# libraz/mygram-db

Hardware: AMD Instinct MI355X
Metric: queries/sec + p50 latency, 10M-doc bigram index, batch=1024 3-term AND (higher is better)
Workload: dtype u32 set algebra + f64 BM25

## Files before the change

### mygram-db_amd/csrc/mgx_api.cpp

```cpp
#include <hip/hip_runtime.h>

#include <dlfcn.h>
#include <pthread.h>

#include <algorithm>
#include <atomic>
#include <chrono>
#include <cmath>
#include <condition_variable>
#include <map>
#include <cstdio>
#include <cstdlib>
#include <cstring>
#include <functional>
#include <memory>
#include <mutex>
#include <string>
#include <thread>
#include <tuple>
#include <unordered_map>
#include <vector>

#include "../../include/mygram_gpu.h"
#include "mgx_highlight.hpp"
// ... 272 lines not shown
    bool operator==(const TableKey& o) const { return row == o.row && idf == o.idf && k1 == o.k1 && b == o.b && avg == o.avg; }
  };
  struct TableKeyHash {
    size_t operator()(const TableKey& k) const {
      uint64_t h = k.row * 0x9E3779B97F4A7C15ull;
      for (uint64_t v : {k.idf, k.k1, k.b, k.avg}) h = (h ^ v) * 0xFF51AFD7ED558CCDull + (h >> 29);
      return static_cast<size_t>(h);
    }
  };
  std::mutex table_mu;
  std::unordered_map<TableKey, uint32_t, TableKeyHash> table_slot;
  DevBuf d_table_pool;
  uint32_t table_cap = 0, table_used = 0, table_dl = 0;
  hipStream_t table_stream = nullptr;
  hipEvent_t table_ev = nullptr;
  mgx::TableJob* job_ring = nullptr;
  DevBuf d_job_ring;
  uint32_t job_ring_at = 0;
  std::vector<mgx::TableJob> pending_jobs;
  hipEvent_t chain_ev = nullptr;
  std::atomic<int> fifo{1};
  bool table_ev_recorded = false;
  static constexpr uint32_t kJobRing = 4096;
  size_t table_doubles() const { return static_cast<size_t>(mgx::kFastPoolTf + 1) * table_dl; }
  struct NormTable {
    uint64_t k1, b, avg;
    DevBuf d;
  };
  std::vector<std::unique_ptr<NormTable>> norm_tables;
  struct BlockMax {
    uint64_t k1, b, avg;
    double step;
    DevBuf d, d_fine;
  };
  std::vector<std::unique_ptr<BlockMax>> block_max;
  std::unordered_map<std::string, uint64_t> df_cache;
  uint32_t n_bitmap_rows = 0, n_fine_rows = 0;
  std::atomic<uint32_t> live_row{mgx::kNoRow};
  std::atomic<bool> bitmaps_clean{false};
  DevBuf d_doc_map;
  DevBuf d_fine_rows;
  std::vector<uint32_t> h_fine_map;
};

namespace mgx {
struct RcclId {
  char internal[128];
};
constexpr int kRcclUint8 = 1, kRcclUint64 = 5, kRcclSum = 0;
static inline uint64_t Bits(double d) {
  uint64_t u;
  std::memcpy(&u, &d, 8);
  return u;
}

static hipError_t SyncDevIndex(mgx_index* idx) {
  if (!idx->d_dev_index.p) {
    ResourceScope none(nullptr);
    hipError_t e = idx->d_dev_index.Alloc(sizeof(DevIndex));
    if (e != hipSuccess) return e;
  }
  return hipMemcpy(idx->d_dev_index.p, &idx->dev, sizeof(DevIndex), hipMemcpyHostToDevice);
}

static uint64_t GetContributionTable(mgx_index* idx, uint32_t bm_row, double idf, double k1, double b, double avgdl) {
  if (idx->table_cap == 0) return 0;
// ... 41 lines not shown
    done += n;
  }
  idx->pending_jobs.clear();
  if ((e = hipEventRecord(idx->table_ev, idx->table_stream)) != hipSuccess) return e;
  idx->table_ev_recorded = true;
  return hipSuccess;
}

static const double* GetLengthNormTable(mgx_index* idx, double k1, double b, double avgdl) {
  std::lock_guard<std::mutex> lock(idx->table_mu);
  for (const auto& t : idx->norm_tables)
    if (t->k1 == Bits(k1) && t->b == Bits(b) && t->avg == Bits(avgdl)) return t->d.as<double>();
  if (idx->norm_tables.size() >= 64) return nullptr;
  double h[256];
  const double one_minus_b = 1.0 - b, avg = std::max(avgdl, 1.0);
  for (uint32_t dli = 0; dli < 256; ++dli) {
    const double length_norm = one_minus_b + b * static_cast<double>(dli) / avg;
    h[dli] = k1 * length_norm;
  }
  auto t = std::make_unique<mgx_index::NormTable>();
  t->k1 = Bits(k1);
  t->b = Bits(b);
  t->avg = Bits(avgdl);
  ResourceScope none(nullptr);
  if (hipSetDevice(idx->device) != hipSuccess || t->d.Alloc(sizeof(h)) != hipSuccess ||
      hipMemcpy(t->d.p, h, sizeof(h), hipMemcpyHostToDevice) != hipSuccess) {
    (void)hipGetLastError();
    return nullptr;
  }
  idx->norm_tables.push_back(std::move(t));
  return idx->norm_tables.back()->d.as<double>();
}

static const uint8_t* GetBlockMax(mgx_index* idx, double k1, double b, double avgdl, double* step, const uint8_t** fine) {
  *fine = nullptr;
  static const bool off = std::getenv("MGX_NO_PRUNE") != nullptr && atoi(std::getenv("MGX_NO_PRUNE")) != 0;
  if (off || !idx->can_score || idx->n_bitmap_rows == 0 || !(k1 > 0.0) || !(b >= 0.0 && b <= 1.0) || !(avgdl >= 0.0))
    return nullptr;
  {
    std::lock_guard<std::mutex> lock(idx->table_mu);
    for (const auto& t : idx->block_max)
      if (t->k1 == Bits(k1) && t->b == Bits(b) && t->avg == Bits(avgdl)) {
        *step = t->step;
        *fine = t->d_fine.as<uint8_t>();
        return t->d.as<uint8_t>();
      }
    if (idx->block_max.size() >= 4) return nullptr;
  }
  const double* ktab = GetLengthNormTable(idx, k1, b, avgdl);
  if (!ktab) return nullptr;
  std::lock_guard<std::mutex> lock(idx->table_mu);
  for (const auto& t : idx->block_max)
    if (t->k1 == Bits(k1) && t->b == Bits(b) && t->avg == Bits(avgdl)) {
      *step = t->step;
      *fine = t->d_fine.as<uint8_t>();
      return t->d.as<uint8_t>();
    }
  auto t = std::make_unique<mgx_index::BlockMax>();
  t->k1 = Bits(k1);
  t->b = Bits(b);
  t->avg = Bits(avgdl);
  t->step = (k1 + 1.0) / 253.0;
  ResourceScope none(nullptr);
  const size_t bytes = static_cast<size_t>(idx->dev.n_tiles) * idx->n_bitmap_rows * 256u;
  if (hipSetDevice(idx->device) != hipSuccess || t->d.Alloc(bytes) != hipSuccess) {
    (void)hipGetLastError();
    return nullptr;
  }
  const size_t fine_bytes = static_cast<size_t>(idx->dev.n_tiles) * idx->n_fine_rows * 1024u;
  if (fine_bytes && t->d_fine.Alloc(fine_bytes) != hipSuccess) {
    (void)hipGetLastError();
    return nullptr;
  }
  if (LaunchBuildBlockMax(idx->dev.tfnib, idx->dev.nib_row_stride, idx->dev.dl8, ktab, k1 + 1.0, 1.0 / t->step, nullptr,
                          idx->n_bitmap_rows, idx->dev.n_tiles, false, t->d.p, idx->stream) != 0 ||
      LaunchBuildBlockMax(idx->dev.tfnib, idx->dev.nib_row_stride, idx->dev.dl8, ktab, k1 + 1.0, 1.0 / t->step,
                          idx->d_fine_rows.as<uint32_t>(), idx->n_fine_rows, idx->dev.n_tiles, true, t->d_fine.p,
                          idx->stream) != 0 ||
      hipStreamSynchronize(idx->stream) != hipSuccess) {
    (void)hipGetLastError();
    return nullptr;
  }
  *step = t->step;
  *fine = t->d_fine.as<uint8_t>();
  idx->block_max.push_back(std::move(t));
  return idx->block_max.back()->d.as<uint8_t>();
}
}


extern "C" {

int mgx_abi_version(void) { return MGX_ABI_VERSION; }
const char* mgx_last_error(void) { return mgx::g_last_error.c_str(); }
void mgx_free(void* p) { std::free(p); }

int mgx_device_count(void) {
  int n = 0;
  if (hipGetDeviceCount(&n) != hipSuccess) {
    (void)hipGetLastError();
    return 0;
  }
  return n;
}


int mgx_columns_build(const mgx_build_params* params, const uint8_t* text_bytes, const uint64_t* text_off,
                      uint32_t first_doc_id, uint64_t n_docs, mgx_columns** out) {
  if (out) *out = nullptr;
  if (!params || !out || !text_off || (n_docs && !text_bytes && text_off[n_docs] != 0))
    return mgx::Fail(MGX_ERR_INVALID_ARGUMENT, "mgx_columns_build: null argument");
  if (params->struct_size < sizeof(mgx_build_params) || params->version != MGX_ABI_VERSION)
    return mgx::Fail(MGX_ERR_INVALID_ARGUMENT, "mgx_columns_build: bad struct_size/version");
  if (static_cast<uint64_t>(first_doc_id) + n_docs > 0xFFFFFFFFull)
    return mgx::Fail(MGX_ERR_OUT_OF_RANGE, "mgx_columns_build: doc ids exceed uint32");
  try {
    mgx::Columns* c = nullptr;
// ... 285 lines not shown
}

void mgx_index_destroy(mgx_index* idx) {
  if (!idx) return;
  (void)hipSetDevice(idx->device);
  if (idx->stream) (void)hipStreamDestroy(idx->stream);
  if (idx->side_stream) (void)hipStreamDestroy(idx->side_stream);
  if (idx->table_stream) {
    (void)hipStreamSynchronize(idx->table_stream);
    (void)hipStreamDestroy(idx->table_stream);
  }
  if (idx->table_ev) (void)hipEventDestroy(idx->table_ev);
  if (idx->job_ring) (void)hipHostFree(idx->job_ring);
  delete idx;
}

int mgx_posting_size(const mgx_index* idx, uint32_t gram_id, uint64_t* out) {
  if (out) *out = 0;
  if (!idx || !out) return mgx::Fail(MGX_ERR_INVALID_ARGUMENT, "mgx_posting_size: null argument");
  if (gram_id >= idx->n_grams) return mgx::Fail(MGX_ERR_OUT_OF_RANGE, "mgx_posting_size: unknown gram id");
  *out = idx->h_offsets[gram_id + 1] - idx->h_offsets[gram_id];
  return MGX_OK;
}

int mgx_index_memory_bytes(const mgx_index* idx, uint64_t* out) {
  if (out) *out = 0;
  if (!idx || !out) return mgx::Fail(MGX_ERR_INVALID_ARGUMENT, "mgx_index_memory_bytes: null argument");
  *out = idx->d_offsets.bytes + idx->d_docids.bytes + idx->d_tf.bytes + idx->d_doc_len.bytes +
         idx->d_skip_row.bytes + idx->d_tile_off.bytes + idx->d_gram_bitmaps.bytes + idx->d_filter_bitmaps.bytes +
         idx->d_text.bytes + idx->d_text_off.bytes + idx->d_dl8.bytes + idx->d_tfnib.bytes + idx->d_table_pool.bytes +
         idx->d_tf_ovf_pos.bytes + idx->d_tf_ovf_val.bytes;
  {
    std::lock_guard<std::mutex> lock(const_cast<mgx_index*>(idx)->table_mu);
    for (const auto& t : idx->block_max) *out += t->d.bytes + t->d_fine.bytes;
    for (const auto& t : idx->norm_tables) *out += t->d.bytes;
  }
  return MGX_OK;
}

int mgx_index_set_batch_order(mgx_index* idx, uint32_t order) {
  if (!idx || order > MGX_ORDER_CONCURRENT) return mgx::Fail(MGX_ERR_INVALID_ARGUMENT, "mgx_index_set_batch_order: bad argument");
  idx->fifo.store(order == MGX_ORDER_FIFO ? 1 : 0);
  return MGX_OK;
}

int mgx_index_attach_text(mgx_index* idx, const uint8_t* text_bytes, const uint64_t* text_off) {
  if (!idx || !text_off) return mgx::Fail(MGX_ERR_INVALID_ARGUMENT, "mgx_index_attach_text: null argument");
  const uint64_t n = idx->dev.n_docs;
  for (uint64_t i = 0; i < n; ++i)
    if (text_off[i + 1] < text_off[i] || text_off[i + 1] - text_off[i] > 0xFFFFFFFFull)
      return mgx::Fail(MGX_ERR_INVALID_ARGUMENT, "mgx_index_attach_text: offsets must ascend");
  const uint64_t total = text_off[n] - text_off[0];
  if (total && !text_bytes) return mgx::Fail(MGX_ERR_INVALID_ARGUMENT, "mgx_index_attach_text: null text");
  std::lock_guard<std::mutex> lock(idx->mu);
  MGX_HIP(hipSetDevice(idx->device));
  std::vector<uint64_t> rel(n + 1);
  for (uint64_t i = 0; i <= n; ++i) rel[i] = text_off[i] - text_off[0];
  MGX_HIP(mgx::Upload(idx->d_text, text_bytes ? text_bytes + text_off[0] : nullptr, total, 128));
  MGX_HIP(mgx::Upload(idx->d_text_off, rel.data(), rel.size()));
  idx->dev.text = idx->d_text.as<uint8_t>();
  idx->dev.text_off = idx->d_text_off.as<uint64_t>();
  uint64_t longest = 0;
  for (uint64_t i = 0; i < n; ++i) longest = std::max<uint64_t>(longest, text_off[i + 1] - text_off[i]);
  idx->max_text_bytes = static_cast<uint32_t>(longest);
  MGX_HIP(mgx::SyncDevIndex(idx));
  return MGX_OK;
}
// ... 1014 lines not shown
    if (f.n_ops == static_cast<uint32_t>(kFastMaxOps) || (op == kOpLoad) != (f.n_ops == 0)) return false;
    FastOp o{};
    uint64_t stride = 0;
    if (lf.kind == kLeafGramBitmap) {
      o.base = reinterpret_cast<uint64_t>(idx->dev.gram_bitmaps + static_cast<uint64_t>(lf.b) * idx->dev.gb_row_stride);
      stride = idx->dev.gb_tile_stride * 8;
    } else if (lf.kind == kLeafFilterBitmap) {
      o.base = static_cast<uint64_t>(lf.b) * idx->dev.fb_row_stride * 8;
      stride = idx->dev.fb_tile_stride * 8;
      o.code |= 16u;
    } else if (lf.kind == kLeafCondBitmap) {
      o.base = reinterpret_cast<uint64_t>(cond_arena + static_cast<uint64_t>(lf.b) * idx->dev.fb_row_stride);
      stride = idx->dev.fb_tile_stride * 8;
    } else {
      return false;
    }
    if (stride > 0xFFFFFFFFull) return false;
    o.tile_stride = static_cast<uint32_t>(stride);
    o.code |= (op == kOpLoad || op == kOpOr) ? kFastOr : op == kOpAnd ? kFastAnd : kFastAndNot;
    f.ops[f.n_ops++] = o;
  }
  if (f.n_ops == 0) return false;
  for (size_t t = 0; t < s.score.size(); ++t) {
    const DevLeaf& lf = s.leaves[s.score[t].leaf];
    if (lf.kind != kLeafGramBitmap) return false;
    FastScore& fs = f.score[t];
    fs.nib = reinterpret_cast<uint64_t>(idx->dev.tfnib + static_cast<uint64_t>(lf.b) * idx->dev.nib_row_stride);
    fs.idf = s.score[t].idf;
    fs.gram = lf.a;
    fs.skip_row = lf.row;
  }
  if (s.reverse != 0) {
    double step = 0.0;
    f.blockmax = GetBlockMax(idx, s.k1, s.b, s.avgdl, &step, &f.blockmax_fine);
    if (f.blockmax) {
      f.bm_tile_stride = idx->n_bitmap_rows * 256u;
      f.bmf_tile_stride = idx->n_fine_rows * 1024u;
      double idf_max = 0.0;
      for (size_t t = 0; t < s.score.size(); ++t) idf_max = std::max(idf_max, s.score[t].idf);
      const double wunit = idf_max > 0.0 ? idf_max * (1.0 + 0x1p-40) / 255.0 : 1.0;
      f.bm_inv_unit = 1.0 / (wunit * step);
      f.bm_wpack = f.bm_w4 = f.bm_cint = 0;
      for (size_t t = 0; t < s.score.size(); ++t) {
        const uint32_t w = static_cast<uint32_t>(std::min(255.0, std::ceil(s.score[t].idf / wunit)));
        if (t < 4) f.bm_wpack |= w << (8 * t); else f.bm_w4 = w;
      }
      for (size_t t = 0; t < s.score.size(); ++t) {
        const DevLeaf& lf = s.leaves[s.score[t].leaf];
        FastScore& fs = f.score[t];
        const uint32_t frow = f.blockmax_fine ? idx->h_fine_map[lf.b] : kNoRow;
        fs.bm_mode = frow != kNoRow ? 2u : 1u;
        fs.bm_off = frow != kNoRow ? frow * 1024u : lf.b * 256u;
      }
    }
  }
  f.n_score = static_cast<uint32_t>(s.score.size());
  f.needed = q.needed;
  f.cap = q.cap;
  f.descending = q.descending;
  f.k1 = q.k1;
  f.b = q.b;
  f.one_minus_b = q.one_minus_b;
  f.k1_plus_1 = q.k1_plus_1;
  f.avgdl_clamped = q.avgdl_clamped;
  return true;
}

static void RouteCandMerge(mgx_batch* b, Group& g, const std::vector<QuerySpec>& specs, const PathSwitches& sw,
                           GroupPlan& p) {
  static const uint64_t kMaxPerTile = std::getenv("MGX_CAND_MAX_PER_TILE") ? static_cast<uint64_t>(atoll(std::getenv("MGX_CAND_MAX_PER_TILE"))) : 64ull;
  const mgx_index* idx = b->idx;
  for (uint32_t i = 0; sw.cand && i < p.n; ++i) {
    const QuerySpec& s = specs[g.qids[i]];
    if (p.route[i] == Route::kFast || !s.flat || s.prog.empty()) continue;
    if (p.score_mode && (!s.fast_score_ok || s.score.empty())) continue;
    bool ok = true, counted = false;
    uint32_t driver = kNoLeaf;
    uint64_t best = ~0ull, longest_list = 0;
    for (size_t pc = 0; ok && pc < s.prog.size(); ++pc) {
      const uint32_t op = s.prog[pc] >> 24, arg = s.prog[pc] & 0xFFFFFFu;
      if (op == kOpCount) {
        counted = true;
        continue;
      }
      if ((op == kOpLoad) != (pc == 0) || (op != kOpLoad && op != kOpAnd && op != kOpAndNot)) { ok = false; break; }
// ... 2559 lines not shown
```

### mygram-db_amd/csrc/mgx_internal.hpp

```cpp
#pragma once

#include <cstdint>

namespace mgx {

constexpr int kBlock = 256;
constexpr int kTileShift = 14;
constexpr uint32_t kTileDocs = 1u << kTileShift;
constexpr int kWordsPerTile = kTileDocs / 64;
constexpr int kMaxTilesPerItem = 64;
constexpr uint32_t kNoRow = 0xFFFFFFFFu;
constexpr uint32_t kMaxLeaves = 192;
constexpr uint32_t kMaxLdsLeaves = 64;
constexpr uint32_t kMaxScoreTerms = 64;
constexpr uint32_t kMaxNeeded = 1024;
constexpr uint32_t kMergeMaxOps = 6;
constexpr uint32_t kMatchBuf = 2048;

enum LeafKind : uint32_t {
  kLeafList = 0,
  kLeafGramBitmap = 1,
  kLeafFilterBitmap = 2,
  kLeafRange = 3,
  kLeafExplicit = 4,
// ... 98 lines not shown
  const uint32_t* tile_off;
  const uint64_t* gram_bitmaps;
  uint64_t gb_tile_stride, gb_row_stride;
  const uint64_t* filter_bitmaps;
  uint64_t fb_tile_stride, fb_row_stride;
  const uint8_t* text;
  const uint64_t* text_off;
  uint32_t first_doc_id;
  uint32_t n_docs;
  uint32_t n_tiles;
  uint32_t max_doc_len;
};

constexpr int kFastMaxOps = 8;
constexpr int kFastMaxScore = 5;
constexpr uint32_t kFastPoolTf = 14;
#ifndef MGX_FWAVES
#define MGX_FWAVES 8
#endif
constexpr int kFastBlock = 64 * MGX_FWAVES;
constexpr int kFastWaves = kFastBlock / 64;

enum FastOpKind : uint32_t { kFastOr = 0, kFastAnd = 1, kFastAndNot = 2 };
struct FastOp {
  uint64_t base;
  uint32_t tile_stride;
  uint32_t code;
};
struct FastScore {
  uint64_t nib;
  double idf;
  uint32_t gram, skip_row;
  uint32_t bm_mode, bm_off;
};
struct DevFastQuery {
  uint32_t n_ops, n_score, needed, cap;
  uint32_t descending, pad0;
  uint32_t pad1, pad1b;
  uint32_t bm_wpack, bm_w4;
  uint32_t bm_cint, pad2;
  double bm_inv_unit;
  double k1, b, one_minus_b, k1_plus_1, avgdl_clamped;
  const uint8_t* blockmax;
  const uint8_t* blockmax_fine;
  uint32_t bm_tile_stride, bmf_tile_stride;
  FastOp ops[kFastMaxOps];
  FastScore score[kFastMaxScore];
};
static_assert(sizeof(DevFastQuery) % 8 == 0, "DevFastQuery is read with scalar loads");

struct FastPlan {
  uint32_t ring;
  uint32_t max_cap;
  uint32_t bytes, pad;
  const double* ktab;
};
struct TableJob {
  double idf, k1, b, avgdl;
  uint32_t slot, pad;
};
FastPlan PlanFast(uint32_t max_cap, const double* ktab);
uint32_t FastTableDl(uint32_t max_doc_len);

struct DevItem {
  uint32_t query, tile_begin, n_tiles, list;
};

struct DevCondition {
  uint64_t literal;
  double eq_epsilon;
  uint32_t op, null_matches, never_matches;
// ... 100 lines not shown
```

### mygram-db_amd/csrc/mgx_kernels.hip

```cpp
#include <hip/hip_runtime.h>

#include <algorithm>
#include <cstdlib>

#include "mgx_fuzzy.hpp"
#include "mgx_internal.hpp"
#include "mgx_launch.hpp"

namespace mgx {

#ifdef MGX_ABLATION
#define MGX_ABLATE(bt, bit) (((bt).debug_skip & (bit)) != 0)
#else
#define MGX_ABLATE(bt, bit) false
#endif


__device__ __forceinline__ int lane_id() { return threadIdx.x & 63; }

__device__ __forceinline__ uint32_t wave_uniform(uint32_t v) { return __builtin_amdgcn_readfirstlane(v); }
__device__ __forceinline__ float wave_uniform(float v) {
  return __uint_as_float(__builtin_amdgcn_readfirstlane(__float_as_uint(v)));
}
__device__ __forceinline__ uint64_t wave_uniform(uint64_t v) {
// ... 116 lines not shown
                                    const uint64_t* __restrict__ row_hi, uint32_t first_doc_id, uint32_t row0,
                                    uint64_t tile_stride, uint64_t row_stride,
                                    unsigned long long* __restrict__ bitmaps) {
  const uint32_t row = blockIdx.y;
  const uint64_t lo = row_lo[row], hi = row_hi[row];
  unsigned long long* bm = bitmaps + static_cast<uint64_t>(row0 + row) * row_stride;
  for (uint64_t p = lo + static_cast<uint64_t>(blockIdx.x) * blockDim.x + threadIdx.x; p < hi;
       p += static_cast<uint64_t>(gridDim.x) * blockDim.x) {
    const uint32_t slot = docids[p] - first_doc_id;
    atomicOr(&bm[static_cast<uint64_t>(slot >> kTileShift) * tile_stride + ((slot >> 6) & (kWordsPerTile - 1))],
             1ull << (slot & 63));
  }
}

__global__ void build_tfnib_kernel(const uint32_t* __restrict__ docids, const uint8_t* __restrict__ tf,
                                   const uint64_t* __restrict__ row_lo, const uint64_t* __restrict__ row_hi,
                                   uint32_t first_doc_id, uint64_t row_stride_bytes, uint8_t* __restrict__ nib) {
  const uint32_t row = blockIdx.y;
  const uint64_t lo = row_lo[row], hi = row_hi[row];
  uint32_t* out = reinterpret_cast<uint32_t*>(nib + static_cast<uint64_t>(row) * row_stride_bytes);
  for (uint64_t p = lo + static_cast<uint64_t>(blockIdx.x) * blockDim.x + threadIdx.x; p < hi;
       p += static_cast<uint64_t>(gridDim.x) * blockDim.x) {
    const uint32_t slot = docids[p] - first_doc_id;
    const uint32_t v = tf[p] < 15 ? tf[p] : 15u;
    atomicOr(&out[slot >> 3], v << ((slot & 7u) * 4u));
  }
}

template <bool kFine>
__global__ __launch_bounds__(256) void build_blockmax_kernel(const uint8_t* __restrict__ nib, uint64_t nib_row_stride,
                                                             const uint8_t* __restrict__ dl8,
                                                             const double* __restrict__ ktab, double k1_plus_1,
                                                             double inv_step, const uint32_t* __restrict__ rows,
                                                             uint32_t n_rows, uint64_t n_out, void* __restrict__ out) {
  const uint64_t idx = static_cast<uint64_t>(blockIdx.x) * blockDim.x + threadIdx.x;
  if (idx >= n_out) return;
  const uint32_t word = static_cast<uint32_t>(idx & 255u);
  const uint64_t tr = idx >> 8;
  const uint32_t r = static_cast<uint32_t>(tr % n_rows);
  const uint32_t row = rows ? rows[r] : r;
  const uint64_t gw = (tr / n_rows) * 256u + word;
  const uint4* np = reinterpret_cast<const uint4*>(nib + static_cast<uint64_t>(row) * nib_row_stride + gw * 32u);
  const uint4* dp = reinterpret_cast<const uint4*>(dl8 + gw * 64u);
  const uint4 n4[2] = {np[0], np[1]};
  const uint4 d4[4] = {dp[0], dp[1], dp[2], dp[3]};
  const uint32_t nw[8] = {n4[0].x, n4[0].y, n4[0].z, n4[0].w, n4[1].x, n4[1].y, n4[1].z, n4[1].w};
  const uint32_t dw[16] = {d4[0].x, d4[0].y, d4[0].z, d4[0].w, d4[1].x, d4[1].y, d4[1].z, d4[1].w,
                           d4[2].x, d4[2].y, d4[2].z, d4[2].w, d4[3].x, d4[3].y, d4[3].z, d4[3].w};
  double best[4] = {0.0, 0.0, 0.0, 0.0};
#pragma unroll
  for (int s = 0; s < 64; ++s) {
    const uint32_t tf = (nw[s >> 3] >> ((s & 7) * 4)) & 15u;
    if (tf == 0u) continue;
    const uint32_t d = (dw[s >> 2] >> ((s & 3) * 8)) & 255u;
    const double tfd = static_cast<double>(tf);
    const double gv = tf == 15u ? k1_plus_1 : tfd * k1_plus_1 / (tfd + ktab[d]);
    best[s >> 4] = gv > best[s >> 4] ? gv : best[s >> 4];
  }
  uint32_t packed = 0, whole = 0;
#pragma unroll
  for (int j = 0; j < 4; ++j) {
    uint32_t qv = 0;
    if (best[j] > 0.0) {
      const double steps = floor(best[j] * inv_step * (1.0 + 0x1p-40));
      qv = steps >= 254.0 ? 255u : static_cast<uint32_t>(steps) + 1u;
    }
    packed |= qv << (8 * j);
    whole = qv > whole ? qv : whole;
  }
  if (kFine) static_cast<uint32_t*>(out)[idx] = packed;
  else static_cast<uint8_t*>(out)[idx] = static_cast<uint8_t>(whole);
}


__device__ __forceinline__ void scatter_segment(const uint32_t* __restrict__ ids, uint64_t lo, uint64_t hi,
                                                uint32_t tile_first_doc, uint32_t* __restrict__ bm32) {
  uint64_t p0 = lo & ~3ull;
  for (uint64_t p = p0 + 4ull * threadIdx.x; p < hi; p += 4ull * kBlock) {
    const uint4 v = *reinterpret_cast<const uint4*>(ids + p);
    const uint32_t e[4] = {v.x, v.y, v.z, v.w};
    uint32_t curw = 0xFFFFFFFFu, curm = 0;
#pragma unroll
    for (int j = 0; j < 4; ++j) {
      uint64_t q = p + j;
      if (q >= lo && q < hi) {
        uint32_t bit = e[j] - tile_first_doc;
        uint32_t w = bit >> 5, m = 1u << (bit & 31);
        if (w == curw) {
          curm |= m;
        } else {
          if (curm) atomicOr(&bm32[curw], curm);
          curw = w;
          curm = m;
        }
      }
    }
    if (curm) atomicOr(&bm32[curw], curm);
  }
}

struct WaveTopK {
  uint64_t* keys;
  uint32_t* docs;
  uint32_t cap, needed;
// ... 1367 lines not shown
__global__ __launch_bounds__(kWaveBlock, 6) void wave_score_lists_kernel(DevIndex ix, DevBatch bt, WavePlan plan) {
  wave_score_body(ix, bt, plan);
}


#ifndef MGX_FPL
#define MGX_FPL 4
#endif
constexpr int kFastPerLane = MGX_FPL;
constexpr uint32_t kFastRound = 64 * kFastPerLane;
constexpr uint32_t kFastPairs = 320;

struct FastOffsets {
  uint32_t ktab, pairs, ring, tk_keys, tk_docs, misc, total;
};
__host__ __device__ inline FastOffsets carve_fast(const FastPlan& p) {
  FastOffsets o;
  uint32_t at = 0;
  o.ktab = at;     at += 256 * 8;
  o.pairs = at;    at += kFastWaves * kFastPairs * 8;
  o.ring = at;     at += kFastWaves * p.ring * 4;
  o.tk_keys = at;  at += kFastWaves * 2 * p.max_cap * 8;
  o.tk_docs = at;  at += kFastWaves * 2 * p.max_cap * 4;
  o.misc = at;     at += 64;
  o.total = at;
  return o;
}
uint32_t FastTableDl(uint32_t max_doc_len) {
  const uint32_t t = max_doc_len + 1 < kTableDlMax ? max_doc_len + 1 : kTableDlMax;
  return (t + 1u) & ~1u;
}
FastPlan PlanFast(uint32_t max_cap, const double* ktab) {
  FastPlan p{};
  p.ring = kFastRound + 128;
  p.max_cap = max_cap;
  p.ktab = ktab;
  p.bytes = carve_fast(p).total;
  return p;
}

typedef uint32_t u32x4 __attribute__((ext_vector_type(4)));
typedef const u32x4 __attribute__((address_space(1)))* gptr_u4;
typedef const uint32_t __attribute__((address_space(1)))* gptr_u1;
typedef const DevFastQuery __attribute__((address_space(4)))* FastQueryPtr;

__device__ __noinline__ uint32_t fast_exact_tf(const DevIndex* ix, uint32_t gram, uint32_t row, uint32_t slot) {
  return exact_tf(*ix, gram, row, slot);
}

template <int T>
__device__ __forceinline__ void fast_load_blockmax(const FastQueryPtr fq, uint32_t tile, uint32_t lane, u32x4 (&raw)[T]) {
  const uint64_t bm = reinterpret_cast<uint64_t>(fq->blockmax), bmf = reinterpret_cast<uint64_t>(fq->blockmax_fine);
  const uint32_t st = fq->bm_tile_stride, stf = fq->bmf_tile_stride;
#pragma unroll
  for (int i = 0; i < T; ++i) {
    const bool fine = fq->score[i].bm_mode == 2u;
    const uint64_t row = (fine ? bmf : bm) + static_cast<uint64_t>(tile) * (fine ? stf : st) + fq->score[i].bm_off;
    const uint32_t off = fine ? lane << 4 : (lane >> 2) << 4;
    raw[i] = *reinterpret_cast<gptr_u4>(row + off);
  }
}

template <int T>
__device__ __forceinline__ uint32_t fast_quarter_mask(const FastQueryPtr fq, uint32_t lane, const u32x4 (&raw)[T],
                                                      uint64_t bound) {
  const uint32_t tint = static_cast<uint32_t>(
      fmin(floor(key_score(bound, true) * fq->bm_inv_unit * (1.0 - 0x1p-30)), 4294967040.0));
  const uint32_t wpack = fq->bm_wpack, w4 = fq->bm_w4, cint = fq->bm_cint;
  uint32_t bmw[T][4];
#pragma unroll
  for (int i = 0; i < T; ++i) {
    bmw[i][0] = raw[i].x;
    bmw[i][1] = raw[i].y;
    bmw[i][2] = raw[i].z;
    bmw[i][3] = raw[i].w;
    const uint32_t mode = fq->score[i].bm_mode;
    if (mode == 1u) {
      const uint32_t l3 = lane & 3u;
      const uint32_t c = l3 == 0u ? raw[i].x : l3 == 1u ? raw[i].y : l3 == 2u ? raw[i].z : raw[i].w;
      bmw[i][0] = __builtin_amdgcn_perm(0u, c, 0x00000000u);
      bmw[i][1] = __builtin_amdgcn_perm(0u, c, 0x01010101u);
      bmw[i][2] = __builtin_amdgcn_perm(0u, c, 0x02020202u);
      bmw[i][3] = __builtin_amdgcn_perm(0u, c, 0x03030303u);
    } else if (mode != 2u) {
      bmw[i][0] = bmw[i][1] = bmw[i][2] = bmw[i][3] = 0;
    }
  }
  uint32_t mk = 0;
#pragma unroll
  for (int k = 0; k < 4; ++k) {
    const uint32_t t0 = bmw[0][k], t1 = T > 1 ? bmw[T > 1 ? 1 : 0][k] : 0u, t2 = T > 2 ? bmw[T > 2 ? 2 : 0][k] : 0u,
                   t3 = T > 3 ? bmw[T > 3 ? 3 : 0][k] : 0u;
    const uint32_t lo01 = __builtin_amdgcn_perm(t1, t0, 0x05010400u), hi01 = __builtin_amdgcn_perm(t1, t0, 0x07030602u);
    const uint32_t lo23 = T > 2 ? __builtin_amdgcn_perm(t3, t2, 0x05010400u) : 0u;
    const uint32_t hi23 = T > 2 ? __builtin_amdgcn_perm(t3, t2, 0x07030602u) : 0u;
    uint32_t qb[4];
    qb[0] = __builtin_amdgcn_perm(lo23, lo01, 0x05040100u);
    qb[1] = __builtin_amdgcn_perm(lo23, lo01, 0x07060302u);
    qb[2] = __builtin_amdgcn_perm(hi23, hi01, 0x05040100u);
    qb[3] = __builtin_amdgcn_perm(hi23, hi01, 0x07060302u);
// ... 33 lines not shown

  WaveTopK tk;
  tk.cap = fq->cap;
  tk.needed = fq->needed;
  tk.lds_sort = true;
  tk.keys = reinterpret_cast<uint64_t*>(smem + fo.tk_keys) + static_cast<size_t>(wave) * 2 * fq->cap;
  tk.docs = reinterpret_cast<uint32_t*>(smem + fo.tk_docs) + static_cast<size_t>(wave) * 2 * fq->cap;
  tk.have = 0;
  tk.pend = 0;
  tk.bound_key = 0;
  tk.bound_doc = 0;
  tk.gbound_ptr = bt.bounds ? bt.bounds + it.query : nullptr;
  tk.gbound = 0;
  for (uint32_t i = lane; i < 2 * tk.cap; i += 64) {
    tk.keys[i] = 0;
    tk.docs[i] = 0;
  }
  __syncthreads();

  __amdgpu_buffer_rsrc_t nib_rsrc[T];
  double idf[T];
#pragma unroll
  for (int i = 0; i < T; ++i) {
    nib_rsrc[i] = __builtin_amdgcn_make_buffer_rsrc(reinterpret_cast<void*>(fq->score[i].nib), 0,
                                                    static_cast<int>((ix.n_docs + 1u) >> 1), 0x00020000);
    idf[i] = fq->score[i].idf;
  }
  const __amdgpu_buffer_rsrc_t dl_rsrc = __builtin_amdgcn_make_buffer_rsrc(
      const_cast<uint8_t*>(ix.dl8), 0, static_cast<int>(ix.n_docs), 0x00020000);
  const double k1_plus_1 = fq->k1_plus_1;
  const bool prune = fq->blockmax != 0;

  uint32_t cnt0 = 0, cnt1 = 0, cnt2 = 0, cnt3 = 0, cnt_res = 0;
  uint32_t pend = 0;
  uint32_t np = 0;

  auto score_round = [&](uint32_t g0, uint32_t n) {
    uint32_t slot[kFastPerLane], dli[kFastPerLane], nb[kFastPerLane][T];
#pragma unroll
    for (int m = 0; m < kFastPerLane; ++m) {
      const uint32_t j = m * 64 + lane;
      slot[m] = j < n ? ring[g0 + j] : 0u;
    }
#pragma unroll
    for (int m = 0; m < kFastPerLane; ++m) {
#pragma unroll
      for (int i = 0; i < T; ++i) nb[m][i] = __builtin_amdgcn_raw_buffer_load_b8(nib_rsrc[i], slot[m] >> 1, 0, 0);
      dli[m] = __builtin_amdgcn_raw_buffer_load_b8(dl_rsrc, slot[m], 0, 0);
    }
#pragma nounroll
    for (int m = 0; m < kFastPerLane; ++m) {
      if (static_cast<uint32_t>(m) * 64u >= n) break;
      uint32_t sl = slot[0], dl = dli[0], nbm[T];
#pragma unroll
      for (int i = 0; i < T; ++i) nbm[i] = nb[0][i];
#pragma unroll
      for (int mm = 1; mm < kFastPerLane; ++mm) {
        if (m == mm) {
          sl = slot[mm];
          dl = dli[mm];
#pragma unroll
          for (int i = 0; i < T; ++i) nbm[i] = nb[mm][i];
        }
      }
      const bool valid = static_cast<uint32_t>(m) * 64u + lane < n;
      double kd = ktab[dl];
      const uint32_t sh = (sl & 1u) << 2;
      uint32_t tf[T], mx = 0;
#pragma unroll
      for (int i = 0; i < T; ++i) {
        tf[i] = (nbm[i] >> sh) & 15u;
        mx = max(mx, tf[i]);
      }
      if (__ballot(valid && (mx == 15u || dl == 255u)) != 0) {
#pragma unroll
        for (int i = 0; i < T; ++i)
          if (valid && tf[i] == 15u) tf[i] = fast_exact_tf(bt.dev_index, fq->score[i].gram, fq->score[i].skip_row, sl);
        if (valid && dl == 255u) {
          const double dld = static_cast<double>(ix.doc_len[sl]);
          kd = fq->k1 * (fq->one_minus_b + fq->b * dld / fq->avgdl_clamped);
        }
      }
      double score = 0.0;
#pragma unroll
      for (int i = 0; i < T; ++i) {
        const double tfd = static_cast<double>(tf[i]);
        const double c = tf[i] != 0u ? idf[i] * (tfd * k1_plus_1) / (tfd + kd) : 0.0;
        score = i == 0 ? c : score + c;
      }
      const uint32_t doc = ix.first_doc_id + sl;
      wave_topk_offer(tk, valid, score_key(score, desc), desc ? doc : ~doc);
    }
  };

  auto load_half = [&](uint32_t o, uint32_t tile, uint32_t h) {
    const uint64_t op_base = fq->ops[o].base;
    const uint32_t op_code = fq->ops[o].code, op_stride = fq->ops[o].tile_stride;
    const uint64_t base = op_base + ((op_code & 16u) ? reinterpret_cast<uint64_t>(ix.filter_bitmaps) : 0ull) +
                          static_cast<uint64_t>(tile) * op_stride;
    const gptr_u4 p = reinterpret_cast<gptr_u4>(base) + lane * 2 + h;
    return p[0];
  };

  for (uint32_t tile = tile_begin + wave;; tile += kFastWaves) {
    const bool flush = tile >= tile_end;
    uint32_t a[8] = {0, 0, 0, 0, 0, 0, 0, 0};
    uint64_t bound = 0;
    if (!flush) {
      wave_topk_refresh_gbound(tk);
      uint32_t qmask = 0xFFFFu;
      if (prune) {
        bound = tk.gbound;
        if (tk.have >= tk.needed && tk.bound_key > bound) bound = tk.bound_key;
      }
      u32x4 raw[T];
#pragma unroll
      for (int i = 0; i < T; ++i) raw[i] = u32x4{0u, 0u, 0u, 0u};
      if (prune) fast_load_blockmax<T>(fq, tile, lane, raw);
      auto combine = [&](int h, uint32_t o, const u32x4 w) {
        const uint32_t code = fq->ops[o].code;
        const uint32_t x[4] = {w.x, w.y, w.z, w.w};
        const uint32_t kind = wave_uniform(code & 15u);
        if (kind == kFastAnd) {
#pragma unroll
          for (int j = 0; j < 4; ++j) a[h * 4 + j] &= x[j];
// ... 79 lines not shown
            }
            np += static_cast<uint32_t>(__popcll(m));
          }
        }
      }
      for (;;) {
        if (np < 64u && !(flush && (np != 0u || pend != 0u))) break;
        const uint32_t take = min(np, 64u);
        wave_lds_sync();
        uint32_t base = 0, bits = 0;
        if (lane < take) {
          const uint2 pv = pairs[np - take + lane];
          base = pv.x;
          bits = pv.y;
        }
        np -= take;
        for (;;) {
          uint32_t n_new;
          const uint32_t my_first = wave_excl_scan_total(static_cast<uint32_t>(__popc(bits)), &n_new);
          bool more = false;
          if (n_new != 0) {
            const uint32_t space = plan.ring - pend;
            uint32_t r = my_first;
            while (bits != 0 && r < space) {
              ring[pend + r] = base + static_cast<uint32_t>(__builtin_ctz(bits));
              bits &= bits - 1;
              ++r;
            }
            more = n_new > space;
            pend = more ? plan.ring : pend + n_new;
            wave_lds_sync();
          }
          const bool fin = flush && !more && np == 0u;
          uint32_t g0 = 0;
          for (;;) {
            const uint32_t n = min(pend - g0, kFastRound);
            if (n == 0 || (n < kFastRound && !fin)) break;
            if (!MGX_ABLATE(bt, 1u)) score_round(g0, n);
#ifdef MGX_ABLATION
            if (MGX_ABLATE(bt, 64u) && lane == 0) cnt3 += n;
#endif
            g0 += n;
            scored = true;
          }
          if (g0 != 0) {
            const uint32_t left = pend - g0;
            uint32_t v[kFastPerLane];
#pragma unroll
            for (int m = 0; m < kFastPerLane; ++m) v[m] = m * 64 + lane < left ? ring[g0 + m * 64 + lane] : 0u;
            wave_lds_sync();
#pragma unroll
            for (int m = 0; m < kFastPerLane; ++m)
              if (m * 64 + lane < left) ring[m * 64 + lane] = v[m];
            pend = left;
            wave_lds_sync();
          }
          if (!more) break;
        }
      }
      if (flush) break;
    }
    if (flush) break;
  }

  {
    uint32_t v[5] = {cnt0, cnt1, cnt2, cnt3, cnt_res};
#pragma unroll
    for (int s = 0; s < 5; ++s) {
      uint32_t x = v[s];
#pragma unroll
      for (int d = 32; d > 0; d >>= 1) x += __shfl_down(x, d, 64);
      if (lane == 0 && x) atomicAdd(&bt.counters[static_cast<uint64_t>(it.query) * 8 + s], (unsigned long long)x);
    }
  }

  wave_topk_truncate(tk);
  if (lane == 0) misc[wave] = tk.have;
  __syncthreads();
  {
    const uint64_t* all_keys = reinterpret_cast<const uint64_t*>(smem + fo.tk_keys);
    const uint32_t* all_docs = reinterpret_cast<const uint32_t*>(smem + fo.tk_docs);
    const uint32_t cap = tk.cap, needed = tk.needed;
    uint32_t have[kFastWaves];
    uint32_t total = 0;
    for (int w = 0; w < kFastWaves; ++w) {
      have[w] = min(misc[w], needed);
      total += have[w];
// ... 1272 lines not shown
    const uint64_t i = base + lane;
    const bool valid = i < n;
    wave_topk_offer(tk, valid, valid ? keys[i] : 0ull, valid ? dprime[i] : 0u);
  }
  wave_topk_truncate(tk);
  const uint32_t have = tk.have < needed ? tk.have : needed;
  for (uint32_t i = lane; i < have; i += 64) {
    cand_keys[static_cast<uint64_t>(gw) * needed + i] = tk.keys[i];
    cand_docs[static_cast<uint64_t>(gw) * needed + i] = tk.docs[i];
  }
  if (lane == 0) cand_n[gw] = have;
}


#define MGX_KCHECK()                                   \
  do {                                                 \
    hipError_t e_ = hipGetLastError();                 \
    if (e_ != hipSuccess) return static_cast<int>(e_); \
  } while (0)

int LaunchBuildTileOff(const uint64_t* offsets, const uint32_t* docids, const uint32_t* rows_gram, uint32_t n_rows,
                       uint32_t n_tiles, uint32_t first_doc_id, uint32_t* tile_off, hipStream_t s) {
  const uint64_t total = static_cast<uint64_t>(n_rows) * (n_tiles + 1);
  if (total == 0) return 0;
  const uint32_t blocks = static_cast<uint32_t>((total + 255) / 256);
  hipLaunchKernelGGL(build_tile_off_kernel, dim3(blocks), dim3(256), 0, s, offsets, docids, rows_gram, n_rows,
                     n_tiles, first_doc_id, tile_off);
  MGX_KCHECK();
  return 0;
}

int LaunchBuildBlockMax(const uint8_t* nib, uint64_t nib_row_stride, const uint8_t* dl8, const double* ktab,
                        double k1_plus_1, double inv_step, const uint32_t* rows, uint32_t n_rows, uint32_t n_tiles,
                        bool fine, void* out, hipStream_t s) {
  const uint64_t n_out = static_cast<uint64_t>(n_tiles) * n_rows * 256u;
  if (n_out == 0) return 0;
  const dim3 grid(static_cast<uint32_t>((n_out + 255) / 256));
  if (fine)
    hipLaunchKernelGGL(build_blockmax_kernel<true>, grid, dim3(256), 0, s, nib, nib_row_stride, dl8, ktab, k1_plus_1,
                       inv_step, rows, n_rows, n_out, out);
  else
    hipLaunchKernelGGL(build_blockmax_kernel<false>, grid, dim3(256), 0, s, nib, nib_row_stride, dl8, ktab, k1_plus_1,
                       inv_step, rows, n_rows, n_out, out);
  MGX_KCHECK();
  return 0;
}

int LaunchBuildTfNib(const uint32_t* docids, const uint8_t* tf, const uint64_t* row_lo, const uint64_t* row_hi,
                     uint32_t n_rows, uint32_t first_doc_id, uint64_t row_stride_bytes, uint8_t* nib, hipStream_t s) {
  for (uint32_t r0 = 0; r0 < n_rows; r0 += 32768) {
    const uint32_t nr = n_rows - r0 < 32768 ? n_rows - r0 : 32768;
    hipLaunchKernelGGL(build_tfnib_kernel, dim3(64, nr), dim3(256), 0, s, docids, tf, row_lo + r0, row_hi + r0,
                       first_doc_id, row_stride_bytes, nib + static_cast<uint64_t>(r0) * row_stride_bytes);
    MGX_KCHECK();
  }
  return 0;
}

int LaunchBuildBitmaps(const uint32_t* docids, const uint64_t* row_lo, const uint64_t* row_hi, uint32_t n_rows,
                       uint32_t first_doc_id, uint32_t first_row, uint64_t tile_stride, uint64_t row_stride,
                       uint64_t* bitmaps, hipStream_t s) {
  if (n_rows == 0) return 0;
  for (uint32_t r0 = 0; r0 < n_rows; r0 += 32768) {
    const uint32_t nr = n_rows - r0 < 32768 ? n_rows - r0 : 32768;
    hipLaunchKernelGGL(build_bitmap_kernel, dim3(64, nr), dim3(256), 0, s, docids, row_lo + r0, row_hi + r0,
                       first_doc_id, first_row + r0, tile_stride, row_stride,
                       reinterpret_cast<unsigned long long*>(bitmaps));
    MGX_KCHECK();
  }
  return 0;
}

int LaunchTileEval(int mode, const DevIndex& ix, const DevBatch& bt, const LdsPlan& plan, hipStream_t s, uint32_t n_plain,
                   uint32_t n_fz) {
  const uint64_t grid = bt.n_items;
  if (grid == 0) return 0;
// ... 741 lines not shown
```

### mygram-db_amd/csrc/mgx_launch.hpp

```cpp
#pragma once
#include <hip/hip_runtime_api.h>

#include "mgx_internal.hpp"

namespace mgx {

int LaunchBuildTileOff(const uint64_t* offsets, const uint32_t* docids, const uint32_t* rows_gram, uint32_t n_rows,
                       uint32_t n_tiles, uint32_t first_doc_id, uint32_t* tile_off, hipStream_t s);
int LaunchBuildBlockMax(const uint8_t* nib, uint64_t nib_row_stride, const uint8_t* dl8, const double* ktab,
                        double k1_plus_1, double inv_step, const uint32_t* rows, uint32_t n_rows, uint32_t n_tiles,
                        bool fine, void* out, hipStream_t s);
int LaunchBuildTfNib(const uint32_t* docids, const uint8_t* tf, const uint64_t* row_lo, const uint64_t* row_hi,
                     uint32_t n_rows, uint32_t first_doc_id, uint64_t row_stride_bytes, uint8_t* nib, hipStream_t s);
int LaunchBuildBitmaps(const uint32_t* docids, const uint64_t* row_lo, const uint64_t* row_hi, uint32_t n_rows,
                       uint32_t first_doc_id, uint32_t first_row, uint64_t tile_stride, uint64_t row_stride,
                       uint64_t* bitmaps, hipStream_t s);
int LaunchTileEval(int mode, const DevIndex& ix, const DevBatch& bt, const LdsPlan& plan, hipStream_t s,
                   uint32_t n_plain = 0xFFFFFFFFu, uint32_t n_fz = 0);
int LaunchWaveScore(const DevIndex& ix, const DevBatch& bt, const WavePlan& plan, hipStream_t s);
int LaunchBitmapScore(uint32_t n_score, const DevIndex& ix, const DevBatch& bt, const FastPlan& plan, hipStream_t s);
int LaunchWavePage(const DevIndex& ix, const DevBatch& bt, const WavePlan& plan, hipStream_t s);
int LaunchWaveCount(const DevIndex& ix, const DevBatch& bt, const WavePlan& plan, bool text_df, hipStream_t s);
int LaunchCand(int mode, const DevIndex& ix, const DevBatch& bt, uint32_t max_leaves, uint32_t max_instr, uint32_t max_cap,
               hipStream_t s);
uint32_t CandLdsBytes(uint32_t max_leaves, uint32_t max_instr, uint32_t max_cap);
int LaunchMergeScore(const DevIndex& ix, const DevBatch& bt, uint32_t max_leaves, uint32_t max_instr, uint32_t max_ops,
                     uint32_t max_cap, hipStream_t s);
uint32_t MergeLdsBytes(uint32_t max_leaves, uint32_t max_instr, uint32_t max_ops, uint32_t max_cap);
int LaunchReadProbe(const void* src, uint64_t bytes, uint32_t* sink, hipStream_t s);

int LaunchMergeTopK(const DevQuery* queries, const uint32_t* query_ids, uint32_t n_slots, uint32_t n_lists,
                    const uint64_t* keys, const uint32_t* docs, const uint32_t* cnt, uint64_t kq, uint64_t kj,
                    uint64_t dj, uint64_t cq, uint64_t cj, uint64_t* top_keys, uint32_t* top_docs, uint32_t* top_n,
                    uint32_t top_stride, uint32_t* page_docs, double* page_scores, uint32_t* page_n,
                    uint32_t page_stride, const uint32_t* list_begin, const unsigned long long* counters,
                    uint64_t* totals_out, hipStream_t s);
int LaunchExportPages(const DevQuery* queries, uint32_t n, uint32_t stride, const uint32_t* page_docs,
                      const uint64_t* totals, uint64_t* blob64, uint32_t* blob32, hipStream_t s);
int LaunchSumTotals(const uint64_t* totals, uint32_t n_shards, uint32_t n_queries, uint64_t pitch, uint64_t* out,
                    hipStream_t s);
int LaunchPackSeedKeys(const uint32_t* list_begin, const uint8_t* has_seed, const uint64_t* cand_keys, const uint32_t* cand_n,
                       uint32_t cand_stride, uint32_t n, uint32_t k, uint64_t* out, hipStream_t s);
int LaunchApplySeedBounds(const uint64_t* all, uint32_t world, uint32_t n, uint32_t k, const DevQuery* queries,
                          unsigned long long* bounds, hipStream_t s);
// ... 44 lines not shown
```

Baseline: 1.074 million.

## Add per-document quantized score bounds to prefilter candidates before full BM25 scoring

Extends the block-max build to also emit a per-document 8-bit quantized upper-bound score for each bitmap gram row. In the fast top-k query kernel, candidates in the ring are first filtered against the current top-k threshold using these per-doc bounds (dot4 over the term weights), and only survivors are compacted and sent to full f64 scoring. The ring is enlarged to hold the compacted pass buffer. This aims to cut the f64 scoring work for docs that cannot enter the top-k, at the cost of extra memory (one byte per doc per row), extra byte loads per candidate, and a more complex round scheduling loop.

```diff
diff --git a/mygram-db_amd/csrc/mgx_api.cpp b/mygram-db_amd/csrc/mgx_api.cpp
--- a/mygram-db_amd/csrc/mgx_api.cpp
+++ b/mygram-db_amd/csrc/mgx_api.cpp
@@ -328,6 +328,7 @@
     uint64_t k1, b, avg;
     double step;
     DevBuf d, d_fine;
+    DevBuf d_doc;
   };
   std::vector<std::unique_ptr<BlockMax>> block_max;
   std::unordered_map<std::string, uint64_t> df_cache;
@@ -435,8 +436,10 @@
   return idx->norm_tables.back()->d.as<double>();
 }
 
-static const uint8_t* GetBlockMax(mgx_index* idx, double k1, double b, double avgdl, double* step, const uint8_t** fine) {
+static const uint8_t* GetBlockMax(mgx_index* idx, double k1, double b, double avgdl, double* step, const uint8_t** fine,
+                                  const uint8_t** qdoc) {
   *fine = nullptr;
+  *qdoc = nullptr;
   static const bool off = std::getenv("MGX_NO_PRUNE") != nullptr && atoi(std::getenv("MGX_NO_PRUNE")) != 0;
   if (off || !idx->can_score || idx->n_bitmap_rows == 0 || !(k1 > 0.0) || !(b >= 0.0 && b <= 1.0) || !(avgdl >= 0.0))
     return nullptr;
@@ -446,6 +449,7 @@
       if (t->k1 == Bits(k1) && t->b == Bits(b) && t->avg == Bits(avgdl)) {
         *step = t->step;
         *fine = t->d_fine.as<uint8_t>();
+        *qdoc = t->d_doc.as<uint8_t>();
         return t->d.as<uint8_t>();
       }
     if (idx->block_max.size() >= 4) return nullptr;
@@ -457,6 +461,7 @@
     if (t->k1 == Bits(k1) && t->b == Bits(b) && t->avg == Bits(avgdl)) {
       *step = t->step;
       *fine = t->d_fine.as<uint8_t>();
+      *qdoc = t->d_doc.as<uint8_t>();
       return t->d.as<uint8_t>();
     }
   auto t = std::make_unique<mgx_index::BlockMax>();
@@ -475,17 +480,25 @@
     (void)hipGetLastError();
     return nullptr;
   }
+  static const bool kDocBound = !(std::getenv("MGX_DOC_BOUND") && atoi(std::getenv("MGX_DOC_BOUND")) == 0);
+  const uint64_t doc_stride = static_cast<uint64_t>(idx->dev.n_tiles) * kTileDocs;
+  if (kDocBound && t->d_doc.Alloc(doc_stride * idx->n_bitmap_rows) != hipSuccess) {
+    (void)hipGetLastError();
+    t->d_doc.Free();
+  }
   if (LaunchBuildBlockMax(idx->dev.tfnib, idx->dev.nib_row_stride, idx->dev.dl8, ktab, k1 + 1.0, 1.0 / t->step, nullptr,
-                          idx->n_bitmap_rows, idx->dev.n_tiles, false, t->d.p, idx->stream) != 0 ||
+                          idx->n_bitmap_rows, idx->dev.n_tiles, false, t->d.p, t->d_doc.as<uint8_t>(), doc_stride,
+                          idx->stream) != 0 ||
       LaunchBuildBlockMax(idx->dev.tfnib, idx->dev.nib_row_stride, idx->dev.dl8, ktab, k1 + 1.0, 1.0 / t->step,
                           idx->d_fine_rows.as<uint32_t>(), idx->n_fine_rows, idx->dev.n_tiles, true, t->d_fine.p,
-                          idx->stream) != 0 ||
+                          nullptr, 0, idx->stream) != 0 ||
       hipStreamSynchronize(idx->stream) != hipSuccess) {
     (void)hipGetLastError();
     return nullptr;
   }
   *step = t->step;
   *fine = t->d_fine.as<uint8_t>();
+  *qdoc = t->d_doc.as<uint8_t>();
   idx->block_max.push_back(std::move(t));
   return idx->block_max.back()->d.as<uint8_t>();
 }
@@ -837,7 +850,7 @@
          idx->d_tf_ovf_pos.bytes + idx->d_tf_ovf_val.bytes;
   {
     std::lock_guard<std::mutex> lock(const_cast<mgx_index*>(idx)->table_mu);
-    for (const auto& t : idx->block_max) *out += t->d.bytes + t->d_fine.bytes;
+    for (const auto& t : idx->block_max) *out += t->d.bytes + t->d_fine.bytes + t->d_doc.bytes;
     for (const auto& t : idx->norm_tables) *out += t->d.bytes;
   }
   return MGX_OK;
@@ -1918,8 +1931,10 @@
   }
   if (s.reverse != 0) {
     double step = 0.0;
-    f.blockmax = GetBlockMax(idx, s.k1, s.b, s.avgdl, &step, &f.blockmax_fine);
+    const uint8_t* qdoc = nullptr;
+    f.blockmax = GetBlockMax(idx, s.k1, s.b, s.avgdl, &step, &f.blockmax_fine, &qdoc);
     if (f.blockmax) {
+      f.doc_bound = qdoc != nullptr;
       f.bm_tile_stride = idx->n_bitmap_rows * 256u;
       f.bmf_tile_stride = idx->n_fine_rows * 1024u;
       double idf_max = 0.0;
@@ -1937,6 +1952,7 @@
         const uint32_t frow = f.blockmax_fine ? idx->h_fine_map[lf.b] : kNoRow;
         fs.bm_mode = frow != kNoRow ? 2u : 1u;
         fs.bm_off = frow != kNoRow ? frow * 1024u : lf.b * 256u;
+        fs.qdoc = qdoc ? reinterpret_cast<uint64_t>(qdoc) + static_cast<uint64_t>(lf.b) * idx->dev.n_tiles * kTileDocs : 0;
       }
     }
   }
diff --git a/mygram-db_amd/csrc/mgx_internal.hpp b/mygram-db_amd/csrc/mgx_internal.hpp
--- a/mygram-db_amd/csrc/mgx_internal.hpp
+++ b/mygram-db_amd/csrc/mgx_internal.hpp
@@ -154,11 +154,13 @@
   double idf;
   uint32_t gram, skip_row;
   uint32_t bm_mode, bm_off;
+  uint64_t qdoc;
 };
 struct DevFastQuery {
   uint32_t n_ops, n_score, needed, cap;
   uint32_t descending, pad0;
-  uint32_t pad1, pad1b;
+  uint32_t doc_bound;
+  uint32_t pad1b;
   uint32_t bm_wpack, bm_w4;
   uint32_t bm_cint, pad2;
   double bm_inv_unit;
diff --git a/mygram-db_amd/csrc/mgx_kernels.hip b/mygram-db_amd/csrc/mgx_kernels.hip
--- a/mygram-db_amd/csrc/mgx_kernels.hip
+++ b/mygram-db_amd/csrc/mgx_kernels.hip
@@ -172,7 +172,8 @@
                                                              const uint8_t* __restrict__ dl8,
                                                              const double* __restrict__ ktab, double k1_plus_1,
                                                              double inv_step, const uint32_t* __restrict__ rows,
-                                                             uint32_t n_rows, uint64_t n_out, void* __restrict__ out) {
+                                                             uint32_t n_rows, uint64_t n_out, void* __restrict__ out,
+                                                             uint8_t* __restrict__ qdoc, uint64_t qdoc_row_stride) {
   const uint64_t idx = static_cast<uint64_t>(blockIdx.x) * blockDim.x + threadIdx.x;
   if (idx >= n_out) return;
   const uint32_t word = static_cast<uint32_t>(idx & 255u);
@@ -187,29 +188,40 @@
   const uint32_t nw[8] = {n4[0].x, n4[0].y, n4[0].z, n4[0].w, n4[1].x, n4[1].y, n4[1].z, n4[1].w};
   const uint32_t dw[16] = {d4[0].x, d4[0].y, d4[0].z, d4[0].w, d4[1].x, d4[1].y, d4[1].z, d4[1].w,
                            d4[2].x, d4[2].y, d4[2].z, d4[2].w, d4[3].x, d4[3].y, d4[3].z, d4[3].w};
-  double best[4] = {0.0, 0.0, 0.0, 0.0};
-#pragma unroll
-  for (int s = 0; s < 64; ++s) {
-    const uint32_t tf = (nw[s >> 3] >> ((s & 7) * 4)) & 15u;
-    if (tf == 0u) continue;
-    const uint32_t d = (dw[s >> 2] >> ((s & 3) * 8)) & 255u;
-    const double tfd = static_cast<double>(tf);
-    const double gv = tf == 15u ? k1_plus_1 : tfd * k1_plus_1 / (tfd + ktab[d]);
-    best[s >> 4] = gv > best[s >> 4] ? gv : best[s >> 4];
-  }
+  uint32_t qw[16];
   uint32_t packed = 0, whole = 0;
 #pragma unroll
   for (int j = 0; j < 4; ++j) {
-    uint32_t qv = 0;
-    if (best[j] > 0.0) {
-      const double steps = floor(best[j] * inv_step * (1.0 + 0x1p-40));
-      qv = steps >= 254.0 ? 255u : static_cast<uint32_t>(steps) + 1u;
-    }
-    packed |= qv << (8 * j);
-    whole = qv > whole ? qv : whole;
-  }
-  if (kFine) static_cast<uint32_t*>(out)[idx] = packed;
-  else static_cast<uint8_t*>(out)[idx] = static_cast<uint8_t>(whole);
+    uint32_t best = 0;
+#pragma unroll
+    for (int s = j * 16; s < j * 16 + 16; ++s) {
+      if ((s & 3) == 0) qw[s >> 2] = 0;
+      const uint32_t tf = (nw[s >> 3] >> ((s & 7) * 4)) & 15u;
+      if (tf == 0u) continue;
+      const uint32_t d = (dw[s >> 2] >> ((s & 3) * 8)) & 255u;
+      const double tfd = static_cast<double>(tf);
+      const double gv = tf == 15u ? k1_plus_1 : tfd * k1_plus_1 / (tfd + ktab[d]);
+      uint32_t qv = 0;
+      if (gv > 0.0) {
+        const double steps = floor(gv * inv_step * (1.0 + 0x1p-40));
+        qv = steps >= 254.0 ? 255u : static_cast<uint32_t>(steps) + 1u;
+      }
+      qw[s >> 2] |= qv << ((s & 3) * 8);
+      best = qv > best ? qv : best;
+    }
+    packed |= best << (8 * j);
+    whole = best > whole ? best : whole;
+  }
+  if (kFine) {
+    static_cast<uint32_t*>(out)[idx] = packed;
+  } else {
+    static_cast<uint8_t*>(out)[idx] = static_cast<uint8_t>(whole);
+    if (qdoc) {
+      uint4* qp = reinterpret_cast<uint4*>(qdoc + static_cast<uint64_t>(row) * qdoc_row_stride + gw * 64u);
+#pragma unroll
+      for (int v = 0; v < 4; ++v) qp[v] = make_uint4(qw[4 * v], qw[4 * v + 1], qw[4 * v + 2], qw[4 * v + 3]);
+    }
+  }
 }
 
 
@@ -1643,7 +1655,7 @@
 }
 FastPlan PlanFast(uint32_t max_cap, const double* ktab) {
   FastPlan p{};
-  p.ring = kFastRound + 128;
+  p.ring = 2 * kFastRound;
   p.max_cap = max_cap;
   p.ktab = ktab;
   p.bytes = carve_fast(p).total;
@@ -1672,11 +1684,14 @@
   }
 }
 
+__device__ __forceinline__ uint32_t fast_theta_int(const FastQueryPtr fq, uint64_t bound) {
+  return static_cast<uint32_t>(fmin(floor(key_score(bound, true) * fq->bm_inv_unit * (1.0 - 0x1p-30)), 4294967040.0));
+}
+
 template <int T>
 __device__ __forceinline__ uint32_t fast_quarter_mask(const FastQueryPtr fq, uint32_t lane, const u32x4 (&raw)[T],
                                                       uint64_t bound) {
-  const uint32_t tint = static_cast<uint32_t>(
-      fmin(floor(key_score(bound, true) * fq->bm_inv_unit * (1.0 - 0x1p-30)), 4294967040.0));
+  const uint32_t tint = fast_theta_int(fq, bound);
   const uint32_t wpack = fq->bm_wpack, w4 = fq->bm_w4, cint = fq->bm_cint;
   uint32_t bmw[T][4];
 #pragma unroll
@@ -1776,7 +1791,8 @@
   const bool prune = fq->blockmax != 0;
 
   uint32_t cnt0 = 0, cnt1 = 0, cnt2 = 0, cnt3 = 0, cnt_res = 0;
-  uint32_t pend = 0;
+  uint32_t pend = 0, pass = 0;
+  const bool doc_bound = prune && fq->doc_bound != 0;
   uint32_t np = 0;
 
   auto score_round = [&](uint32_t g0, uint32_t n) {
@@ -1835,6 +1851,40 @@
       const uint32_t doc = ix.first_doc_id + sl;
       wave_topk_offer(tk, valid, score_key(score, desc), desc ? doc : ~doc);
     }
+  };
+
+  auto filter_round = [&](uint32_t u0, uint32_t n, uint32_t tint) {
+    uint32_t slot[kFastPerLane], qb[kFastPerLane][T];
+#pragma unroll
+    for (int m = 0; m < kFastPerLane; ++m) {
+      const uint32_t j = m * 64 + lane;
+      slot[m] = j < n ? ring[u0 + j] : 0u;
+    }
+#pragma unroll
+    for (int i = 0; i < T; ++i) {
+      const __amdgpu_buffer_rsrc_t q_rsrc = __builtin_amdgcn_make_buffer_rsrc(
+          reinterpret_cast<void*>(fq->score[i].qdoc), 0, static_cast<int>(ix.n_tiles * kTileDocs), 0x00020000);
+#pragma unroll
+      for (int m = 0; m < kFastPerLane; ++m) qb[m][i] = __builtin_amdgcn_raw_buffer_load_b8(q_rsrc, slot[m], 0, 0);
+    }
+    const uint32_t wpack = fq->bm_wpack, w4 = fq->bm_w4, cint = fq->bm_cint;
+    wave_lds_sync();
+#pragma unroll
+    for (int m = 0; m < kFastPerLane; ++m) {
+      uint32_t packed = qb[m][0];
+      if (T > 1) packed |= qb[m][T > 1 ? 1 : 0] << 8;
+      if (T > 2) packed |= qb[m][T > 2 ? 2 : 0] << 16;
+      if (T > 3) packed |= qb[m][T > 3 ? 3 : 0] << 24;
+      uint32_t ub = __builtin_amdgcn_udot4(packed, wpack, cint, false);
+      if (T > 4) ub += w4 * qb[m][T > 4 ? 4 : 0];
+      const bool keep = static_cast<uint32_t>(m) * 64u + lane < n && ub >= tint;
+      const uint64_t km = __ballot(keep);
+      if (keep)
+        ring[pass + __builtin_amdgcn_mbcnt_hi(static_cast<uint32_t>(km >> 32),
+                                              __builtin_amdgcn_mbcnt_lo(static_cast<uint32_t>(km), 0u))] = slot[m];
+      pass += static_cast<uint32_t>(__popcll(km));
+    }
+    wave_lds_sync();
   };
 
   auto load_half = [&](uint32_t o, uint32_t tile, uint32_t h) {
@@ -1980,27 +2030,53 @@
             wave_lds_sync();
           }
           const bool fin = flush && !more && np == 0u;
-          uint32_t g0 = 0;
+          uint32_t u0 = pass;
           for (;;) {
-            const uint32_t n = min(pend - g0, kFastRound);
-            if (n == 0 || (n < kFastRound && !fin)) break;
-            if (!MGX_ABLATE(bt, 1u)) score_round(g0, n);
+            const uint32_t n1 = min(pend - u0, kFastRound);
+            const bool do1 = n1 == kFastRound || (fin && n1 != 0u);
+            uint32_t g0 = 0, n = 0;
+            if (do1) {
+              uint64_t th = 0;
+              if (doc_bound && !MGX_ABLATE(bt, 128u)) {
+                wave_topk_refresh_gbound(tk);
+                th = tk.gbound;
+                if (tk.have >= tk.needed && tk.bound_key > th) th = tk.bound_key;
+              }
+              if (th != 0) {
+                filter_round(u0, n1, fast_theta_int(fq, th));
 #ifdef MGX_ABLATION
-            if (MGX_ABLATE(bt, 64u) && lane == 0) cnt3 += n;
+                if (MGX_ABLATE(bt, 256u) && lane == 0) cnt3 += n1;
 #endif
-            g0 += n;
-            scored = true;
+              } else {
+                g0 = u0;
+                n = n1;
+              }
+              u0 += n1;
+            }
+            if (n == 0 && (pass >= kFastRound / 2 || (fin && u0 == pend))) {
+              n = min(pass, kFastRound);
+              pass -= n;
+              g0 = pass;
+            }
+            if (n != 0) {
+              if (!MGX_ABLATE(bt, 1u)) score_round(g0, n);
+#ifdef MGX_ABLATION
+              if (MGX_ABLATE(bt, 64u) && lane == 0) cnt3 += n;
+#endif
+              scored = true;
+            }
+            if (!do1 && n == 0) break;
           }
-          if (g0 != 0) {
-            const uint32_t left = pend - g0;
+          if (u0 != pass) {
+            const uint32_t left = pend - u0;
             uint32_t v[kFastPerLane];
 #pragma unroll
-            for (int m = 0; m < kFastPerLane; ++m) v[m] = m * 64 + lane < left ? ring[g0 + m * 64 + lane] : 0u;
+            for (int m = 0; m < kFastPerLane; ++m) v[m] = m * 64 + lane < left ? ring[u0 + m * 64 + lane] : 0u;
             wave_lds_sync();
 #pragma unroll
             for (int m = 0; m < kFastPerLane; ++m)
-              if (m * 64 + lane < left) ring[m * 64 + lane] = v[m];
-            pend = left;
+              if (m * 64 + lane < left) ring[pass + m * 64 + lane] = v[m];
+            pend = pass + left;
             wave_lds_sync();
           }
           if (!more) break;
@@ -3339,16 +3415,16 @@
 
 int LaunchBuildBlockMax(const uint8_t* nib, uint64_t nib_row_stride, const uint8_t* dl8, const double* ktab,
                         double k1_plus_1, double inv_step, const uint32_t* rows, uint32_t n_rows, uint32_t n_tiles,
-                        bool fine, void* out, hipStream_t s) {
+                        bool fine, void* out, uint8_t* qdoc, uint64_t qdoc_row_stride, hipStream_t s) {
   const uint64_t n_out = static_cast<uint64_t>(n_tiles) * n_rows * 256u;
   if (n_out == 0) return 0;
   const dim3 grid(static_cast<uint32_t>((n_out + 255) / 256));
   if (fine)
     hipLaunchKernelGGL(build_blockmax_kernel<true>, grid, dim3(256), 0, s, nib, nib_row_stride, dl8, ktab, k1_plus_1,
-                       inv_step, rows, n_rows, n_out, out);
+                       inv_step, rows, n_rows, n_out, out, nullptr, 0);
   else
     hipLaunchKernelGGL(build_blockmax_kernel<false>, grid, dim3(256), 0, s, nib, nib_row_stride, dl8, ktab, k1_plus_1,
-                       inv_step, rows, n_rows, n_out, out);
+                       inv_step, rows, n_rows, n_out, out, qdoc, qdoc_row_stride);
   MGX_KCHECK();
   return 0;
 }
diff --git a/mygram-db_amd/csrc/mgx_launch.hpp b/mygram-db_amd/csrc/mgx_launch.hpp
--- a/mygram-db_amd/csrc/mgx_launch.hpp
+++ b/mygram-db_amd/csrc/mgx_launch.hpp
@@ -9,7 +9,7 @@
                        uint32_t n_tiles, uint32_t first_doc_id, uint32_t* tile_off, hipStream_t s);
 int LaunchBuildBlockMax(const uint8_t* nib, uint64_t nib_row_stride, const uint8_t* dl8, const double* ktab,
                         double k1_plus_1, double inv_step, const uint32_t* rows, uint32_t n_rows, uint32_t n_tiles,
-                        bool fine, void* out, hipStream_t s);
+                        bool fine, void* out, uint8_t* qdoc, uint64_t qdoc_row_stride, hipStream_t s);
 int LaunchBuildTfNib(const uint32_t* docids, const uint8_t* tf, const uint64_t* row_lo, const uint64_t* row_hi,
                      uint32_t n_rows, uint32_t first_doc_id, uint64_t row_stride_bytes, uint8_t* nib, hipStream_t s);
 int LaunchBuildBitmaps(const uint32_t* docids, const uint64_t* row_lo, const uint64_t* row_hi, uint32_t n_rows,
```

Measured after the change: 1.031 million. 0.96x the previous value.
